# cc-ai/MUNIT

Measured on AMD Instinct MI355X. Metric: images/sec (gen_update+dis_update) @256x256 bs=8, higher is better.
Workload: dtype f32; 1 GPU; config_256.yaml AdaINGen_double+MsImageDis dis_update+gen_update, 256x256, per-GPU batch 8, fp32; global_batch=8, parallelism=dp1, gen_state=1

## Files before the change

### include/munit_hip.h

```cpp
#ifndef MUNIT_HIP_H
#define MUNIT_HIP_H

#include <stddef.h>
#include <stdint.h>

#ifdef __cplusplus
extern "C" {
#endif

typedef void* munit_stream_t;

enum { MUNIT_OK = 0, MUNIT_ERR_ARG = -1, MUNIT_ERR_WORKSPACE = -2, MUNIT_ERR_LAUNCH = -3 };
enum { MUNIT_ACT_NONE = 0, MUNIT_ACT_RELU = 1, MUNIT_ACT_LRELU = 2, MUNIT_ACT_TANH = 3 };
enum { MUNIT_PAD_ZERO = 0, MUNIT_PAD_REFLECT = 1 };
enum { MUNIT_COMPUTE_F32 = 0, MUNIT_COMPUTE_BF16 = 1, MUNIT_COMPUTE_F32X3 = 2 };
enum { MUNIT_DTYPE_F32 = 0, MUNIT_DTYPE_BF16 = 1 };

int munit_version(void);
const char* munit_last_error(void);

typedef void* munit_comm_t;
int munit_comm_unique_id(void* id_out, size_t bytes);
int munit_comm_init(munit_comm_t* comm, int rank, int world, const void* unique_id);
int munit_comm_allreduce(munit_comm_t comm, float* buf, size_t count, munit_stream_t stream);
int munit_comm_destroy(munit_comm_t comm);
int munit_shutdown(void);

int munit_stream_wait_stream(munit_stream_t waiter, munit_stream_t signaler);

typedef struct {
  int B, H, W, Cin;
  int Cout, KH, KW;
  int stride, pad, pad_mode;
  int upsample;
  int act;
  float slope;
  int compute;
  int in_dtype, out_dtype;
} munit_conv_desc;

int munit_conv2d_out_hw(const munit_conv_desc* d, int* Ho, int* Wo);

size_t munit_conv2d_fwd_workspace_bytes(const munit_conv_desc* d);
int munit_conv2d_fwd(const munit_conv_desc* d, const void* x, const float* w, const float* bias,
                     void* y, void* ws, size_t ws_bytes, munit_stream_t stream);

size_t munit_conv2d_dgrad_workspace_bytes(const munit_conv_desc* d);
int munit_conv2d_dgrad(const munit_conv_desc* d, const void* dy, const float* w, const void* add,
                       void* dx, void* ws, size_t ws_bytes, munit_stream_t stream);

size_t munit_conv2d_wgrad_workspace_bytes(const munit_conv_desc* d);
int munit_conv2d_wgrad(const munit_conv_desc* d, const void* x, const void* dy, float* dw,
                       float* db, float beta, void* ws, size_t ws_bytes, munit_stream_t stream);

enum { MUNIT_PASS_FWD = 0, MUNIT_PASS_DGRAD = 1, MUNIT_PASS_WGRAD = 2 };
enum { MUNIT_PREP_NONE = 0, MUNIT_PREP_DGRAD = 1, MUNIT_PREP_SUBPIXEL = 2, MUNIT_PREP_CAST = 3,
       MUNIT_PREP_WINOGRAD = 4, MUNIT_PREP_WINOGRAD_DGRAD = 5, MUNIT_PREP_SUBPIXEL_WINOGRAD = 6,
       MUNIT_PREP_WINOGRAD_S2 = 7, MUNIT_PREP_WINOGRAD_S2_DGRAD = 8,
       MUNIT_PREP_SUBPIXEL_WINOGRAD_DGRAD = 9  };
typedef struct {
  const float* w;
  float* wp;
  int Cout, KH, KW, Cin;
  int kind;
  int ps;
  int bf16;
} munit_prep_item;
size_t munit_conv2d_prepared_weight_bytes(const munit_conv_desc* d, int pass);
int munit_conv2d_prep_item(const munit_conv_desc* d, int pass, const float* w, float* wp, munit_prep_item* out);
int munit_conv2d_prepare_weights(const munit_prep_item* item, munit_stream_t stream);
int munit_conv2d_prepare_weights_batch(const munit_prep_item* items_dev, int n, munit_stream_t stream);
int munit_conv2d_fwd_prepared(const munit_conv_desc* d, const void* x, const float* w, const void* wp,
                              const float* bias, void* y, void* ws, size_t ws_bytes, munit_stream_t stream);
int munit_conv2d_dgrad_prepared(const munit_conv_desc* d, const void* dy, const float* w, const void* wp,
                                const void* add, void* dx, void* ws, size_t ws_bytes, munit_stream_t stream);

size_t munit_linear_workspace_bytes(int B, int K, int N);
int munit_linear_fwd(const float* x, const float* w, const float* bias, float* y, int B, int K, int N, int act,
                     float slope, void* ws, size_t ws_bytes, munit_stream_t stream);
int munit_linear_bwd(const float* x, const float* w, const float* dy, float* dx, float* dw, float* db, int B, int K,
                     int N, float beta, void* ws, size_t ws_bytes, munit_stream_t stream);

double munit_conv2d_executed_flops(const munit_conv_desc* d, int pass);
const char* munit_conv2d_kernel_name(const munit_conv_desc* d, int pass);

int munit_act_bwd(int act, float slope, const float* y, const float* dy, float* dx, size_t n,
                  munit_stream_t stream);

size_t munit_instnorm_workspace_bytes(int B, int HW, int C);
int munit_instnorm_fwd(const float* x, float* y, float* stats, int B, int HW, int C,
                       const float* adain, int ad_ld, int w_off, int b_off, const float* residual,
                       int relu, float eps, void* ws, size_t ws_bytes, munit_stream_t stream);
int munit_instnorm_bwd(const float* x, const float* dy, const float* stats, float* dx, int B, int HW,
                       int C, const float* adain, float* d_adain, int ad_ld, int w_off, int b_off,
                       int relu, void* ws, size_t ws_bytes, munit_stream_t stream);

int munit_instnorm_fwd_bf16(const void* x, void* y, float* stats, int B, int HW, int C,
                            const float* adain, int ad_ld, int w_off, int b_off, const void* residual,
                            int relu, float eps, void* ws, size_t ws_bytes, munit_stream_t stream);
int munit_instnorm_bwd_bf16(const void* x, const void* dy, const float* stats, void* dx, int B, int HW,
                            int C, const float* adain, float* d_adain, int ad_ld, int w_off, int b_off,
                            int relu, void* ws, size_t ws_bytes, munit_stream_t stream);

size_t munit_layernorm_workspace_bytes(int B, int HW, int C);
int munit_layernorm_fwd(const float* x, float* y, float* stats, int B, int HW, int C,
                        const float* gamma, const float* beta, int relu, float eps, void* ws,
                        size_t ws_bytes, munit_stream_t stream);
int munit_layernorm_bwd(const float* x, const float* dy, const float* stats, float* dx, int B, int HW,
                        int C, const float* gamma, const float* beta, float* dgamma, float* dbeta,
                        float acc, int relu, float eps, void* ws, size_t ws_bytes,
                        munit_stream_t stream);

int munit_layernorm_fwd_bf16(const void* x, void* y, float* stats, int B, int HW, int C,
                             const float* gamma, const float* beta, int relu, float eps, void* ws,
                             size_t ws_bytes, munit_stream_t stream);
int munit_layernorm_bwd_bf16(const void* x, const void* dy, const float* stats, void* dx, int B, int HW,
                             int C, const float* gamma, const float* beta, float* dgamma, float* dbeta,
                             float acc, int relu, float eps, void* ws, size_t ws_bytes,
                             munit_stream_t stream);

int munit_avgpool3s2_fwd(const float* x, float* y, int B, int H, int W, int C, munit_stream_t stream);
int munit_avgpool3s2_bwd(const float* dy, float* dx, int B, int H, int W, int C, munit_stream_t stream);
int munit_gap_fwd(const float* x, float* y, int B, int HW, int C, munit_stream_t stream);
int munit_gap_bwd(const float* dy, float* dx, int B, int HW, int C, munit_stream_t stream);

size_t munit_loss_workspace_bytes(size_t n);
int munit_l1_mean_fwd(const float* a, const float* b, const float* mask, size_t npix, int C, float* out,
                      void* ws, size_t ws_bytes, munit_stream_t stream);
int munit_l1_mean_bwd(const float* a, const float* b, const float* mask, size_t npix, int C,
                      const float* gout, float* da, float* db, munit_stream_t stream);
int munit_l1_mean_fwd_bf16(const void* a, const void* b, const float* mask, size_t npix, int C, float* out,
                           void* ws, size_t ws_bytes, munit_stream_t stream);
int munit_l1_mean_bwd_bf16(const void* a, const void* b, const float* mask, size_t npix, int C,
                           const float* gout, void* da, void* db, munit_stream_t stream);
int munit_pair_l1_fwd(const float* x_a, const float* x_b, const float* x_ab, const float* x_ba, size_t npix, int C,
                      float* out, void* ws, size_t ws_bytes, munit_stream_t stream);
int munit_pair_l1_bwd(const float* x_a, const float* x_b, const float* x_ab, const float* x_ba, size_t npix, int C,
                      const float* gout, float* dx_ab, float* dx_ba, munit_stream_t stream);
int munit_mse_const_fwd(const float* x, float target, size_t n, float* out, void* ws, size_t ws_bytes,
                        munit_stream_t stream);
int munit_mse_const_bwd(const float* x, float target, size_t n, const float* gout, float* dx,
                        munit_stream_t stream);
size_t munit_lsgan_workspace_bytes(int nseg);
int munit_lsgan_fwd(const float* const* x, const size_t* n, const float* target, int nseg, float* out, float* seg_out,
                    void* ws, size_t ws_bytes, munit_stream_t stream);
int munit_lsgan_bwd(const float* const* x, const size_t* n, const float* target, int nseg, const float* gout,
                    float* const* dx, munit_stream_t stream);
size_t munit_nsgan_workspace_bytes(int nseg);
int munit_nsgan_fwd(const float* const* x, const size_t* n, const float* target, int nseg, float* out, float* seg_out,
                    void* ws, size_t ws_bytes, munit_stream_t stream);
int munit_nsgan_bwd(const float* const* x, const size_t* n, const float* target, int nseg, const float* gout,
                    float* const* dx, munit_stream_t stream);
int munit_weighted_sum(const float* const* terms, const float* w, int n, float* out,
                       munit_stream_t stream);

int munit_adam_step(float* p, const float* g, float* m, float* v, size_t n, double lr, double beta1,
                    double beta2, double eps, double weight_decay, int step, munit_stream_t stream);

int munit_extraadam_step(float* p, const float* g, float* m, float* v, float* p_saved, size_t n, double lr,
                         double beta1, double beta2, double eps, double weight_decay, int step, int mode,
                         munit_stream_t stream);

int munit_scale(const float* x, float* y, size_t n, float alpha, int accumulate, munit_stream_t stream);

typedef struct {
  long long src_off;
  int src_h, src_w;
  int rs_h, rs_w;
  int crop_i, crop_j;
  int flip;
  int kind;
} munit_image_desc;

int munit_image_ksize(int src_size, int rs_size);
size_t munit_image_preprocess_workspace_bytes(int B, int out_h, int out_w, int ksize_max);
int munit_image_preprocess(const unsigned char* pool, const munit_image_desc* descs, int B, int out_h,
                           int out_w, int ksize_max, float* out, void* ws, size_t ws_bytes,
                           munit_stream_t stream);
// ... 109 lines not shown
```

### munit_amd/_lib.py

```python
import ctypes
import os
from ctypes import POINTER, Structure, c_char_p, c_double, c_float, c_int, c_size_t, c_void_p

_HERE = os.path.dirname(os.path.abspath(__file__))
LIB_PATH = os.environ.get("MUNIT_HIP_LIB") or os.path.join(_HERE, "libmunit_hip.so")

ACT = {"none": 0, "relu": 1, "lrelu": 2, "tanh": 3}
PAD = {"zero": 0, "reflect": 1}
COMPUTE = {"f32": 0, "bf16": 1, "f32x3": 2}
DTYPE = {"f32": 0, "bf16": 1}


class ConvDesc(Structure):
    _fields_ = [("B", c_int), ("H", c_int), ("W", c_int), ("Cin", c_int),
                ("Cout", c_int), ("KH", c_int), ("KW", c_int),
                ("stride", c_int), ("pad", c_int), ("pad_mode", c_int),
                ("upsample", c_int), ("act", c_int), ("slope", c_float), ("compute", c_int),
                ("in_dtype", c_int), ("out_dtype", c_int)]


class PrepItem(Structure):
    _fields_ = [("w", c_void_p), ("wp", c_void_p), ("Cout", c_int), ("KH", c_int), ("KW", c_int), ("Cin", c_int),
                ("kind", c_int), ("ps", c_int), ("bf16", c_int)]


class ImageDesc(Structure):
    _fields_ = [("src_off", ctypes.c_longlong), ("src_h", c_int), ("src_w", c_int), ("rs_h", c_int), ("rs_w", c_int),
                ("crop_i", c_int), ("crop_j", c_int), ("flip", c_int), ("kind", c_int)]


class GemmProblem(Structure):
    _fields_ = [("A", c_void_p), ("B", c_void_p), ("C", c_void_p)]


class GridSrc(Structure):
    _fields_ = [("data", c_void_p), ("n", c_int), ("channels", c_int), ("layout", c_int)]


class RectDesc(Structure):
    _fields_ = [("B", c_int), ("H", c_int), ("W", c_int), ("Cin", c_int), ("x_ld", c_int), ("Cout", c_int), ("y_ld", c_int),
                ("KH", c_int), ("KW", c_int), ("stride", c_int), ("pad_h", c_int), ("pad_w", c_int), ("relu", c_int)]


WINDOW = {"max": 0, "avg": 1}
RECT_TILES = ("128x128", "64x64", "128x64")

_P = c_void_p
_DESC = POINTER(ConvDesc)

SIGNATURES = {
    "munit_version": (c_int, []),
    "munit_last_error": (c_char_p, []),
    "munit_stream_wait_stream": (c_int, [_P, _P]),
    "munit_comm_unique_id": (c_int, [_P, c_size_t]),
    "munit_comm_init": (c_int, [_P, c_int, c_int, _P]),
    "munit_comm_allreduce": (c_int, [_P, _P, c_size_t, _P]),
    "munit_comm_destroy": (c_int, [_P]),
    "munit_shutdown": (c_int, []),
    "munit_conv2d_out_hw": (c_int, [_DESC, POINTER(c_int), POINTER(c_int)]),
    "munit_conv2d_fwd_workspace_bytes": (c_size_t, [_DESC]),
    "munit_conv2d_fwd": (c_int, [_DESC, _P, _P, _P, _P, _P, c_size_t, _P]),
    "munit_conv2d_dgrad_workspace_bytes": (c_size_t, [_DESC]),
    "munit_conv2d_dgrad": (c_int, [_DESC, _P, _P, _P, _P, _P, c_size_t, _P]),
    "munit_conv2d_wgrad_workspace_bytes": (c_size_t, [_DESC]),
    "munit_conv2d_wgrad": (c_int, [_DESC, _P, _P, _P, _P, c_float, _P, c_size_t, _P]),
    "munit_conv2d_prepared_weight_bytes": (c_size_t, [_DESC, c_int]),
    "munit_conv2d_prep_item": (c_int, [_DESC, c_int, _P, _P, POINTER(PrepItem)]),
    "munit_conv2d_prepare_weights": (c_int, [POINTER(PrepItem), _P]),
    "munit_conv2d_prepare_weights_batch": (c_int, [_P, c_int, _P]),
    "munit_conv2d_fwd_prepared": (c_int, [_DESC, _P, _P, _P, _P, _P, _P, c_size_t, _P]),
    "munit_conv2d_dgrad_prepared": (c_int, [_DESC, _P, _P, _P, _P, _P, _P, c_size_t, _P]),
    "munit_conv2d_executed_flops": (c_double, [_DESC, c_int]),
    "munit_conv2d_kernel_name": (c_char_p, [_DESC, c_int]),
    "munit_linear_workspace_bytes": (c_size_t, [c_int, c_int, c_int]),
    "munit_linear_fwd": (c_int, [_P, _P, _P, _P, c_int, c_int, c_int, c_int, c_float, _P, c_size_t, _P]),
    "munit_linear_bwd": (c_int, [_P, _P, _P, _P, _P, _P, c_int, c_int, c_int, c_float, _P, c_size_t, _P]),
    "munit_act_bwd": (c_int, [c_int, c_float, _P, _P, _P, c_size_t, _P]),
    "munit_instnorm_workspace_bytes": (c_size_t, [c_int, c_int, c_int]),
    "munit_instnorm_fwd": (c_int, [_P, _P, _P, c_int, c_int, c_int, _P, c_int, c_int, c_int, _P, c_int,
                                   c_float, _P, c_size_t, _P]),
    "munit_instnorm_bwd": (c_int, [_P, _P, _P, _P, c_int, c_int, c_int, _P, _P, c_int, c_int, c_int, c_int,
                                   _P, c_size_t, _P]),
    "munit_instnorm_fwd_bf16": (c_int, [_P, _P, _P, c_int, c_int, c_int, _P, c_int, c_int, c_int, _P, c_int,
                                        c_float, _P, c_size_t, _P]),
    "munit_instnorm_bwd_bf16": (c_int, [_P, _P, _P, _P, c_int, c_int, c_int, _P, _P, c_int, c_int, c_int, c_int,
                                        _P, c_size_t, _P]),
    "munit_layernorm_workspace_bytes": (c_size_t, [c_int, c_int, c_int]),
    "munit_layernorm_fwd": (c_int, [_P, _P, _P, c_int, c_int, c_int, _P, _P, c_int, c_float, _P, c_size_t, _P]),
    "munit_layernorm_bwd": (c_int, [_P, _P, _P, _P, c_int, c_int, c_int, _P, _P, _P, _P, c_float, c_int,
                                    c_float, _P, c_size_t, _P]),
    "munit_layernorm_fwd_bf16": (c_int, [_P, _P, _P, c_int, c_int, c_int, _P, _P, c_int, c_float, _P, c_size_t, _P]),
    "munit_layernorm_bwd_bf16": (c_int, [_P, _P, _P, _P, c_int, c_int, c_int, _P, _P, _P, _P, c_float, c_int,
                                         c_float, _P, c_size_t, _P]),
    "munit_avgpool3s2_fwd": (c_int, [_P, _P, c_int, c_int, c_int, c_int, _P]),
    "munit_avgpool3s2_bwd": (c_int, [_P, _P, c_int, c_int, c_int, c_int, _P]),
    "munit_gap_fwd": (c_int, [_P, _P, c_int, c_int, c_int, _P]),
    "munit_gap_bwd": (c_int, [_P, _P, c_int, c_int, c_int, _P]),
    "munit_loss_workspace_bytes": (c_size_t, [c_size_t]),
    "munit_l1_mean_fwd": (c_int, [_P, _P, _P, c_size_t, c_int, _P, _P, c_size_t, _P]),
    "munit_l1_mean_bwd": (c_int, [_P, _P, _P, c_size_t, c_int, _P, _P, _P, _P]),
    "munit_l1_mean_fwd_bf16": (c_int, [_P, _P, _P, c_size_t, c_int, _P, _P, c_size_t, _P]),
    "munit_l1_mean_bwd_bf16": (c_int, [_P, _P, _P, c_size_t, c_int, _P, _P, _P, _P]),
    "munit_pair_l1_fwd": (c_int, [_P, _P, _P, _P, c_size_t, c_int, _P, _P, c_size_t, _P]),
    "munit_pair_l1_bwd": (c_int, [_P, _P, _P, _P, c_size_t, c_int, _P, _P, _P, _P]),
    "munit_mse_const_fwd": (c_int, [_P, c_float, c_size_t, _P, _P, c_size_t, _P]),
    "munit_mse_const_bwd": (c_int, [_P, c_float, c_size_t, _P, _P, _P]),
    "munit_lsgan_workspace_bytes": (c_size_t, [c_int]),
    "munit_lsgan_fwd": (c_int, [POINTER(c_void_p), POINTER(c_size_t), POINTER(c_float), c_int, _P, _P, _P, c_size_t, _P]),
    "munit_lsgan_bwd": (c_int, [POINTER(c_void_p), POINTER(c_size_t), POINTER(c_float), c_int, _P, POINTER(c_void_p), _P]),
    "munit_nsgan_workspace_bytes": (c_size_t, [c_int]),
    "munit_nsgan_fwd": (c_int, [POINTER(c_void_p), POINTER(c_size_t), POINTER(c_float), c_int, _P, _P, _P, c_size_t, _P]),
    "munit_nsgan_bwd": (c_int, [POINTER(c_void_p), POINTER(c_size_t), POINTER(c_float), c_int, _P, POINTER(c_void_p), _P]),
    "munit_weighted_sum": (c_int, [POINTER(c_void_p), POINTER(c_float), c_int, _P, _P]),
    "munit_adam_step": (c_int, [_P, _P, _P, _P, c_size_t, c_double, c_double, c_double, c_double, c_double, c_int,
                                _P]),
    "munit_extraadam_step": (c_int, [_P, _P, _P, _P, _P, c_size_t, c_double, c_double, c_double, c_double,
                                     c_double, c_int, c_int, _P]),
    "munit_scale": (c_int, [_P, _P, c_size_t, c_float, c_int, _P]),
    "munit_image_ksize": (c_int, [c_int, c_int]),
    "munit_image_preprocess_workspace_bytes": (c_size_t, [c_int, c_int, c_int, c_int]),
    "munit_image_preprocess": (c_int, [_P, _P, c_int, c_int, c_int, c_int, _P, _P, c_size_t, _P]),
    "munit_mask_preprocess_workspace_bytes": (c_size_t, [c_int, c_int, c_int]),
    "munit_mask_preprocess": (c_int, [_P, _P, c_int, c_int, c_int, _P, _P, c_size_t, _P]),
    "munit_label_preprocess_workspace_bytes": (c_size_t, [c_int, c_int, c_int]),
    "munit_label_preprocess": (c_int, [_P, _P, c_int, c_int, c_int, _P, _P, c_size_t, _P]),
    "munit_image_grid_workspace_bytes": (c_size_t, [c_int, c_int, c_int, c_int]),
    "munit_image_grid_u8": (c_int, [POINTER(GridSrc), c_int, c_int, c_int, c_int, c_float, c_float, _P, _P, c_size_t, _P]),
    "munit_seg_input_fwd": (c_int, [_P, _P, c_size_t, _P]),
    "munit_seg_input_bwd": (c_int, [_P, _P, c_size_t, _P]),
    "munit_space_to_batch": (c_int, [_P, _P, c_int, c_int, c_int, c_int, c_int, c_int, _P]),
    "munit_maxpool3s2_fwd": (c_int, [_P, _P, _P, c_int, c_int, c_int, c_int, _P]),
    "munit_maxpool3s2_bwd": (c_int, [_P, _P, _P, c_int, c_int, c_int, c_int, _P]),
    "munit_add_relu_fwd": (c_int, [_P, _P, _P, c_size_t, _P]),
    "munit_seg_ce_workspace_bytes": (c_size_t, [c_int, c_int, c_int, c_int]),
    "munit_seg_ce_fwd": (c_int, [_P, _P, _P, c_int, c_int, c_int, c_int, c_float, _P, _P, c_size_t, _P]),
    "munit_seg_ce_bwd": (c_int, [_P, _P, _P, c_int, c_int, c_int, c_int, c_float, _P, _P, _P, c_size_t, _P]),
    "munit_seg_ce_gt_fwd": (c_int, [_P, _P, _P, c_int, c_int, c_int, c_int, c_float, _P, _P, c_size_t, _P]),
    "munit_seg_ce_gt_bwd": (c_int, [_P, _P, _P, c_int, c_int, c_int, c_int, c_float, _P, _P, _P, c_size_t, _P]),
    "munit_seg_labels": (c_int, [_P, c_int, c_int, c_int, c_int, _P, _P]),
    "munit_seg_ce_direct_workspace_bytes": (c_size_t, [c_int, c_int, c_int, c_int, c_int]),
    "munit_seg_ce_direct_fwd": (c_int, [_P, _P, c_int, c_int, c_int, c_int, c_int, c_float, _P, _P, c_size_t, _P]),
    "munit_seg_ce_direct_bwd": (c_int, [_P, _P, c_int, c_int, c_int, c_int, c_int, c_float, _P, _P, _P, c_size_t, _P]),
    "munit_avgpool7_fwd": (c_int, [_P, _P, c_int, c_int, c_int, c_int, _P]),
    "munit_avgpool7_bwd": (c_int, [_P, _P, c_int, c_int, c_int, c_int, _P]),
    "munit_batchnorm_workspace_bytes": (c_size_t, [c_int]),
    "munit_batchnorm_fwd": (c_int, [_P, _P, _P, _P, _P, _P, ctypes.c_longlong, c_int, _P, _P, c_int, c_int, c_float, c_float,
                                    _P, c_size_t, _P]),
    "munit_batchnorm_bwd": (c_int, [_P, _P, _P, _P, _P, _P, _P, _P, _P, c_float, ctypes.c_longlong, c_int, c_int, _P,
                                    c_size_t, _P]),
    "munit_batchnorm_dp_workspace_bytes": (c_size_t, [c_int]),
    "munit_batchnorm_dp_stats_local": (c_int, [_P, ctypes.c_longlong, c_int, c_int, c_int, _P, c_size_t, _P, c_size_t, _P]),
    "munit_batchnorm_dp_fwd_apply": (c_int, [_P, _P, _P, _P, _P, _P, ctypes.c_longlong, c_int, c_int, _P, c_size_t, _P, _P,
                                             c_int, c_float, c_float, _P]),
    "munit_batchnorm_dp_bwd_local": (c_int, [_P, _P, _P, _P, _P, ctypes.c_longlong, c_int, c_int, c_int, c_int, _P, c_size_t,
                                             _P, c_size_t, _P]),
    "munit_batchnorm_dp_bwd_finish": (c_int, [_P, _P, _P, _P, _P, _P, _P, _P, _P, c_float, ctypes.c_longlong, c_int, c_int,
                                              c_int, c_int, _P, c_size_t, _P, c_size_t, _P]),
    "munit_maxpool2_fwd": (c_int, [_P, _P, _P, c_int, c_int, c_int, c_int, _P]),
    "munit_maxpool2_bwd": (c_int, [_P, _P, _P, c_int, c_int, c_int, c_int, _P]),
    "munit_avgpool16_fwd": (c_int, [_P, _P, c_int, c_int, c_int, c_int, _P]),
    "munit_avgpool16_bwd": (c_int, [_P, _P, c_int, c_int, c_int, c_int, _P]),
# ... 43 lines not shown
```

### munit_amd/csrc/norm.hip

```cpp
#include "common.h"

namespace {

constexpr int NT = 256;
constexpr int MAX_SPLIT = 64;
constexpr int MAX_NORM_C = 4 * NT;

constexpr float NORM_LRELU_SLOPE = 0.2f;
__device__ inline float norm_act(float v, int act) {
  if (act == MUNIT_ACT_RELU) return v > 0.f ? v : 0.f;
  if (act == MUNIT_ACT_LRELU) return v > 0.f ? v : v * NORM_LRELU_SLOPE;
  if (act == MUNIT_ACT_TANH) return tanhf(v);
  return v;
}
__device__ inline float norm_act_grad(float pre, float g, int act) {
  if (act == MUNIT_ACT_RELU) return pre > 0.f ? g : 0.f;
  if (act == MUNIT_ACT_LRELU) return pre > 0.f ? g : g * NORM_LRELU_SLOPE;
  if (act == MUNIT_ACT_TANH) { const float t = tanhf(pre); return g * (1.f - t * t); }
  return g;
}

struct Lay {
  int CQ;
  int QB;
// ... 310 lines not shown
    const float rstd = (float)(1.0 / sqrt(var + (double)eps));
    float w = 1.f, bb = 0.f;
    if (adain != nullptr) {
      w = adain[(long long)b * ad_ld + w_off + c];
      bb = adain[(long long)b * ad_ld + b_off + c];
    }
    if (sp == 0) {
      stats[((long long)b * C + c) * 2] = mean;
      stats[((long long)b * C + c) * 2 + 1] = rstd;
    }
    scale[threadIdx.x] = rstd * w;
    shift[threadIdx.x] = bb - mean * rstd * w;
  }
  __syncthreads();
  const int per = (HW + nsplit - 1) / nsplit;
  const int p0 = sp * per, p1 = min(HW, p0 + per);
  const long long base = (long long)b * HW * C + c0;
  const int q = threadIdx.x & 15;
  const f32x4 sc = *reinterpret_cast<const f32x4*>(scale + q * 4);
  const f32x4 sh = *reinterpret_cast<const f32x4*>(shift + q * 4);
#pragma unroll 4
  for (int p = p0 + (threadIdx.x >> 4); p < p1; p += NT / 16) {
    const long long o = base + (long long)p * C + q * 4;
    f32x4 v = ld4(x + o);
    v = v * sc + sh;
    if (relu) {
#pragma unroll
      for (int e = 0; e < 4; ++e) v[e] = norm_act(v[e], relu);
    }
    if (residual != nullptr) v += ld4(residual + o);
    st4(y + o, v);
  }
}

template <typename T>
__global__ __launch_bounds__(NT) void in_bwd_apply_sliced_kernel(const T* __restrict__ x, const T* __restrict__ dy,
                                                                 const double* __restrict__ partial,
                                                                 const float* __restrict__ stats, T* __restrict__ dx, int HW,
                                                                 int C, int nsplit, const float* __restrict__ adain,
                                                                 float* __restrict__ d_adain, int ad_ld, int w_off, int b_off,
                                                                 int relu) {
  __shared__ double red[3][SLICE][2];
  __shared__ __attribute__((aligned(16))) float s_co[6][SLICE];
  const int b = blockIdx.y, sp = blockIdx.x, c0 = blockIdx.z * SLICE;
  double a1, a2;
  fold_slice(partial, b, C, nsplit, c0, red, a1, a2);
  if (threadIdx.x < SLICE) {
    const int c = c0 + threadIdx.x;
    if (d_adain != nullptr && sp == 0) {
      d_adain[(long long)b * ad_ld + w_off + c] = (float)a2;
      d_adain[(long long)b * ad_ld + b_off + c] = (float)a1;
    }
    const double inv_n = 1.0 / (double)HW;
    s_co[0][threadIdx.x] = stats[((long long)b * C + c) * 2];
    s_co[1][threadIdx.x] = stats[((long long)b * C + c) * 2 + 1];
    s_co[2][threadIdx.x] = adain ? adain[(long long)b * ad_ld + w_off + c] : 1.f;
    s_co[3][threadIdx.x] = adain ? adain[(long long)b * ad_ld + b_off + c] : 0.f;
    s_co[4][threadIdx.x] = (float)(a1 * inv_n);
    s_co[5][threadIdx.x] = (float)(a2 * inv_n);
  }
  __syncthreads();
  const int per = (HW + nsplit - 1) / nsplit;
  const int p0 = sp * per, p1 = min(HW, p0 + per);
  const long long base = (long long)b * HW * C + c0;
  const int q = threadIdx.x & 15;
  const f32x4 mean = *reinterpret_cast<const f32x4*>(&s_co[0][q * 4]);
  const f32x4 rstd = *reinterpret_cast<const f32x4*>(&s_co[1][q * 4]);
  const f32x4 w = *reinterpret_cast<const f32x4*>(&s_co[2][q * 4]);
  const f32x4 bb = *reinterpret_cast<const f32x4*>(&s_co[3][q * 4]);
  const f32x4 a1v = *reinterpret_cast<const f32x4*>(&s_co[4][q * 4]);
  const f32x4 a2v = *reinterpret_cast<const f32x4*>(&s_co[5][q * 4]);
#pragma unroll 4
  for (int p = p0 + (threadIdx.x >> 4); p < p1; p += NT / 16) {
    const long long o = base + (long long)p * C + q * 4;
    const f32x4 xv = ld4(x + o);
    const f32x4 xh = (xv - mean) * rstd;
    f32x4 g = ld4(dy + o);
    if (relu) {
#pragma unroll
      for (int e = 0; e < 4; ++e) g[e] = norm_act_grad(xv[e] * (rstd[e] * w[e]) + (bb[e] - mean[e] * rstd[e] * w[e]), g[e], relu);
    }
    const f32x4 r = rstd * w * (g - a1v - xh * a2v);
    st4(dx + o, r);
  }
}

__device__ inline double block_sum(double v, double* red) {
#pragma unroll
  for (int off = 32; off > 0; off >>= 1) v += __shfl_xor(v, off, 64);
  const int w = threadIdx.x >> 6;
  __syncthreads();
  if ((threadIdx.x & 63) == 0) red[w] = v;
  __syncthreads();
  double t = 0.0;
#pragma unroll
  for (int i = 0; i < NT / 64; ++i) t += red[i];
  return t;
}

template <typename T>
__global__ __launch_bounds__(NT) void ln_stats_kernel(const T* __restrict__ x, double* __restrict__ partial,
                                                      long long n_per_sample, int nsplit) {
  __shared__ double red[NT / 64];
  const int b = blockIdx.y, sp = blockIdx.x;
  const T* xb = x + (long long)b * n_per_sample;
  const long long nq = n_per_sample >> 2;
  const long long per = (nq + nsplit - 1) / nsplit;
  const long long q0 = sp * per, q1 = min(nq, q0 + per);
  const float piv = ld1(xb);
  double s1 = 0.0, s2 = 0.0;
  for (long long i = q0 + threadIdx.x; i < q1; i += NT) {
    f32x4 v = ld4(xb + i * 4);
#pragma unroll
    for (int e = 0; e < 4; ++e) {
      double d = (double)(v[e] - piv);
      s1 += d;
      s2 += d * d;
    }
  }
  s1 = block_sum(s1, red);
  s2 = block_sum(s2, red);
  if (threadIdx.x == 0) {
    partial[((long long)b * nsplit + sp) * 2] = s1;
    partial[((long long)b * nsplit + sp) * 2 + 1] = s2;
  }
}

template <typename T>
__device__ inline void ln_finish(const double* partial, const T* xb, int b, int nsplit, long long n,
                                 float* mean, float* sigma) {
  double s1 = 0.0, s2 = 0.0;
  for (int k = 0; k < nsplit; ++k) {
    s1 += partial[((long long)b * nsplit + k) * 2];
    s2 += partial[((long long)b * nsplit + k) * 2 + 1];
  }
  const double d = s1 / (double)n;
  double var = (s2 - s1 * d) / (double)(n - 1);
  if (var < 0.0) var = 0.0;
  *mean = (float)((double)ld1(xb) + d);
  *sigma = (float)sqrt(var);
}

template <typename T>
__global__ __launch_bounds__(NT) void ln_apply_kernel(const T* __restrict__ x, T* __restrict__ y,
                                                      const double* __restrict__ partial, float* __restrict__ stats,
                                                      int HW, int C, int nsplit, const float* __restrict__ gamma,
                                                      const float* __restrict__ beta, int relu, float eps) {
  extern __shared__ float sm[];
  float* scale = sm;
  float* shift = sm + C;
  const int b = blockIdx.y, sp = blockIdx.x;
  const long long n = (long long)HW * C;
  const T* xb = x + (long long)b * n;
  float mean, sigma;
  ln_finish(partial, xb, b, nsplit, n, &mean, &sigma);
  const float inv = 1.f / (sigma + eps);
  if (sp == 0 && threadIdx.x == 0) {
    stats[b * 2] = mean;
    stats[b * 2 + 1] = sigma;
  }
  for (int c = threadIdx.x; c < C; c += NT) {
    scale[c] = inv * gamma[c];
    shift[c] = beta[c] - mean * inv * gamma[c];
  }
  __syncthreads();
  const int CQ = C >> 2;
// ... 62 lines not shown
    __syncthreads();
    if (pl == 0) {
      for (int l = 1; l < L.PL; ++l) {
        const double* d = sm + ((l * L.QB + q) * 8);
#pragma unroll
        for (int e = 0; e < 4; ++e) { s1[e] += d[e]; s2[e] += d[4 + e]; }
      }
      double* o = cpart + ((long long)(b * nsplit + sp) * 2) * C + qq * 4;
#pragma unroll
      for (int e = 0; e < 4; ++e) { o[e] = s1[e]; o[C + e] = s2[e]; }
    }
    __syncthreads();
  }
  t1 = block_sum(t1, red);
  t2 = block_sum(t2, red);
  if (threadIdx.x == 0) {
    spart[((long long)b * nsplit + sp) * 2] = t1;
    spart[((long long)b * nsplit + sp) * 2 + 1] = t2;
  }
}

template <typename T>
__global__ __launch_bounds__(NT) void ln_bwd_apply_kernel(const T* __restrict__ x, const T* __restrict__ dy,
                                                          const float* __restrict__ stats,
                                                          const double* __restrict__ spart, T* __restrict__ dx,
                                                          int HW, int C, int nsplit, const float* __restrict__ gamma,
                                                          const float* __restrict__ beta, int relu, float eps) {
  const int b = blockIdx.y, sp = blockIdx.x;
  const long long n = (long long)HW * C;
  const float mean = stats[b * 2];
  const float sigma = stats[b * 2 + 1];
  const float inv = 1.f / (sigma + eps);
  double S1 = 0.0, S2 = 0.0;
  for (int k = 0; k < nsplit; ++k) {
    S1 += spart[((long long)b * nsplit + k) * 2];
    S2 += spart[((long long)b * nsplit + k) * 2 + 1];
  }
  const float c1 = (float)(S1 / (double)n);
  const float c2 = sigma > 0.f ? (float)(S2 / ((double)(n - 1) * (double)sigma)) : 0.f;
  const int CQ = C >> 2;
  const long long nq = n >> 2;
  const long long per = (nq + nsplit - 1) / nsplit;
  const long long q0 = sp * per, q1 = min(nq, q0 + per);
  const long long base = (long long)b * n;
  for (long long i = q0 + threadIdx.x; i < q1; i += NT) {
    const int q = (int)(i % CQ);
    const f32x4 gm = *reinterpret_cast<const f32x4*>(gamma + q * 4);
    const f32x4 bt = *reinterpret_cast<const f32x4*>(beta + q * 4);
    const f32x4 xv = ld4(x + base + i * 4);
    const f32x4 xn = (xv - mean) * inv;
    f32x4 g = ld4(dy + base + i * 4);
    if (relu) {
#pragma unroll
      for (int e = 0; e < 4; ++e) g[e] = norm_act_grad(xv[e] * (inv * gm[e]) + (bt[e] - mean * inv * gm[e]), g[e], relu);
    }
    const f32x4 r = (g * gm - c1) * inv - xn * c2;
    st4(dx + base + i * 4, r);
  }
}

__global__ __launch_bounds__(NT) void ln_bwd_param_kernel(const double* __restrict__ cpart, float* __restrict__ dgamma,
                                                          float* __restrict__ dbeta, int C, int nblk, float acc) {
  __shared__ double red[NT / 64];
  const int c = blockIdx.x;
  double g = 0.0, bt = 0.0;
  for (int k = threadIdx.x; k < nblk; k += NT) {
    g += cpart[((long long)k * 2) * C + c];
    bt += cpart[((long long)k * 2 + 1) * C + c];
  }
  g = block_sum(g, red);
  bt = block_sum(bt, red);
  if (threadIdx.x == 0) {
    dgamma[c] = (acc != 0.f ? acc * dgamma[c] : 0.f) + (float)g;
    dbeta[c] = (acc != 0.f ? acc * dbeta[c] : 0.f) + (float)bt;
  }
}

}

namespace {
size_t in_partial_bytes(int B, int C) { return align_up((size_t)B * MAX_SPLIT * 2 * C * sizeof(double), 256); }
bool in_sliced(int C) { return C % SLICE == 0 && !MUNIT_ENV_FLAG("MUNIT_DEBUG_NO_SLICED_NORM"); }
int sliced_split(int B, int HW, int C) { return std::max(1, pick_split(B, HW) / (C / SLICE)); }
}
extern "C" size_t munit_instnorm_workspace_bytes(int B, int HW, int C) {
  return in_partial_bytes(B, C) + align_up((size_t)B * 6 * C * sizeof(float), 256);
}

namespace {
template <typename T>
int instnorm_fwd_t(const T* x, T* y, float* stats, int B, int HW, int C, const float* adain, int ad_ld, int w_off,
                   int b_off, const T* residual, int relu, float eps, void* ws, size_t ws_bytes, munit_stream_t stream) {
  MUNIT_CHECK_ARG(x && y && stats && ws, "instnorm_fwd: null pointer");
  MUNIT_CHECK_ARG(B > 0 && HW > 0 && C > 0 && C % 4 == 0, "instnorm_fwd: bad dims B=%d HW=%d C=%d", B, HW, C);
  MUNIT_CHECK_ARG(C <= MAX_NORM_C, "instnorm_fwd: C=%d too large", C);
  if (ws_bytes < munit_instnorm_workspace_bytes(B, HW, C)) {
    munit_set_error("instnorm_fwd: workspace too small");
    return MUNIT_ERR_WORKSPACE;
  }
  hipStream_t st = (hipStream_t)stream;
  double* partial = reinterpret_cast<double*>(ws);
  if (in_sliced(C)) {
    const int ns = sliced_split(B, HW, C);
    const Lay Ls = make_lay(SLICE);
    hipLaunchKernelGGL(in_stats_kernel<T>, dim3(ns, B, C / SLICE), dim3(NT), (size_t)Ls.PL * Ls.QB * 8 * sizeof(double), st, x,
                       partial, HW, C, ns, SLICE);
    MUNIT_CHECK_LAUNCH("in_stats");
    hipLaunchKernelGGL(in_apply_sliced_kernel<T>, dim3(ns, B, C / SLICE), dim3(NT), 0, st, x, y, partial, stats, HW, C, ns, adain,
                       ad_ld, w_off, b_off, eps, residual, relu);
    MUNIT_CHECK_LAUNCH("in_apply_sliced");
    return MUNIT_OK;
  }
  const int ns = pick_split(B, HW);
  const Lay L = make_lay(C);
  hipLaunchKernelGGL(in_stats_kernel<T>, dim3(ns, B), dim3(NT), (size_t)L.PL * L.QB * 8 * sizeof(double), st, x,
                     partial, HW, C, ns, C);
  MUNIT_CHECK_LAUNCH("in_stats");
  float* coef = reinterpret_cast<float*>(reinterpret_cast<char*>(ws) + in_partial_bytes(B, C));
  hipLaunchKernelGGL(in_finalize_kernel<T>, dim3(cdiv(C, 64), B), dim3(NT), 0, st, x, partial, stats, coef, B,
                     HW, C, ns, adain, ad_ld, w_off, b_off, eps);
  MUNIT_CHECK_LAUNCH("in_finalize");
  hipLaunchKernelGGL(in_apply_kernel<T>, dim3(ns, B), dim3(NT), (size_t)2 * C * sizeof(float), st, x, y, coef, HW, C,
                     ns, residual, relu);
  MUNIT_CHECK_LAUNCH("in_apply");
  return MUNIT_OK;
}

template <typename T>
int instnorm_bwd_t(const T* x, const T* dy, const float* stats, T* dx, int B, int HW, int C, const float* adain,
                   float* d_adain, int ad_ld, int w_off, int b_off, int relu, void* ws, size_t ws_bytes,
                   munit_stream_t stream) {
  MUNIT_CHECK_ARG(x && dy && stats && dx && ws, "instnorm_bwd: null pointer");
  MUNIT_CHECK_ARG(B > 0 && HW > 0 && C > 0 && C % 4 == 0 && C <= MAX_NORM_C, "instnorm_bwd: bad dims");
  if (ws_bytes < munit_instnorm_workspace_bytes(B, HW, C)) {
    munit_set_error("instnorm_bwd: workspace too small");
    return MUNIT_ERR_WORKSPACE;
  }
  hipStream_t st = (hipStream_t)stream;
  double* partial = reinterpret_cast<double*>(ws);
  if (in_sliced(C)) {
    const int ns = sliced_split(B, HW, C);
    const Lay Ls = make_lay(SLICE);
    hipLaunchKernelGGL(in_bwd_stats_kernel<T>, dim3(ns, B, C / SLICE), dim3(NT), (size_t)Ls.PL * Ls.QB * 8 * sizeof(double), st, x,
                       dy, stats, partial, HW, C, ns, adain, ad_ld, w_off, b_off, relu, SLICE);
    MUNIT_CHECK_LAUNCH("in_bwd_stats");
    hipLaunchKernelGGL(in_bwd_apply_sliced_kernel<T>, dim3(ns, B, C / SLICE), dim3(NT), 0, st, x, dy, partial, stats, dx, HW, C, ns,
                       adain, d_adain, ad_ld, w_off, b_off, relu);
    MUNIT_CHECK_LAUNCH("in_bwd_apply_sliced");
    return MUNIT_OK;
  }
  const int ns = pick_split(B, HW);
  const Lay L = make_lay(C);
  hipLaunchKernelGGL(in_bwd_stats_kernel<T>, dim3(ns, B), dim3(NT), (size_t)L.PL * L.QB * 8 * sizeof(double), st, x,
                     dy, stats, partial, HW, C, ns, adain, ad_ld, w_off, b_off, relu, C);
  MUNIT_CHECK_LAUNCH("in_bwd_stats");
  float* coef = reinterpret_cast<float*>(reinterpret_cast<char*>(ws) + in_partial_bytes(B, C));
  hipLaunchKernelGGL(in_bwd_finalize_kernel, dim3(cdiv(C, 64), B), dim3(NT), 0, st, partial, stats, coef, B, HW,
                     C, ns, adain, d_adain, ad_ld, w_off, b_off);
  MUNIT_CHECK_LAUNCH("in_bwd_finalize");
  hipLaunchKernelGGL(in_bwd_apply_kernel<T>, dim3(ns, B), dim3(NT), (size_t)6 * C * sizeof(float), st, x, dy, coef, dx,
                     HW, C, ns, relu);
  MUNIT_CHECK_LAUNCH("in_bwd_apply");
  return MUNIT_OK;
}
}

extern "C" int munit_instnorm_fwd(const float* x, float* y, float* stats, int B, int HW, int C,
                                  const float* adain, int ad_ld, int w_off, int b_off, const float* residual,
                                  int relu, float eps, void* ws, size_t ws_bytes, munit_stream_t stream) {
  return instnorm_fwd_t<float>(x, y, stats, B, HW, C, adain, ad_ld, w_off, b_off, residual, relu, eps, ws, ws_bytes, stream);
}
extern "C" int munit_instnorm_fwd_bf16(const void* x, void* y, float* stats, int B, int HW, int C,
                                       const float* adain, int ad_ld, int w_off, int b_off, const void* residual,
                                       int relu, float eps, void* ws, size_t ws_bytes, munit_stream_t stream) {
  return instnorm_fwd_t<bf16_t>(reinterpret_cast<const bf16_t*>(x), reinterpret_cast<bf16_t*>(y), stats, B, HW, C, adain, ad_ld,
                                w_off, b_off, reinterpret_cast<const bf16_t*>(residual), relu, eps, ws, ws_bytes, stream);
}
extern "C" int munit_instnorm_bwd(const float* x, const float* dy, const float* stats, float* dx, int B, int HW,
                                  int C, const float* adain, float* d_adain, int ad_ld, int w_off, int b_off,
                                  int relu, void* ws, size_t ws_bytes, munit_stream_t stream) {
  return instnorm_bwd_t<float>(x, dy, stats, dx, B, HW, C, adain, d_adain, ad_ld, w_off, b_off, relu, ws, ws_bytes, stream);
}
extern "C" int munit_instnorm_bwd_bf16(const void* x, const void* dy, const float* stats, void* dx, int B, int HW,
                                       int C, const float* adain, float* d_adain, int ad_ld, int w_off, int b_off,
// ... 88 lines not shown
```

Baseline: 79.14 images/s.

## Add single-kernel register-resident instance norm forward for small f32 planes

Adds a one-pass instance-norm forward kernel for f32. Each block handles 16 channels of one image, holds the spatial values in registers, computes shifted double-precision sums, reduces them in shared memory and applies the scale/shift, ReLU and residual in the same launch. This replaces the separate stats and apply kernels, removing one launch and a second read of x when the plane fits. It also adds a route query function. The cost is heavy register use (16 f32x4 per thread) and use only where the split and HW limits hold.

```diff
diff --git a/include/munit_hip.h b/include/munit_hip.h
--- a/include/munit_hip.h
+++ b/include/munit_hip.h
@@ -94,6 +94,8 @@
 int munit_instnorm_bwd(const float* x, const float* dy, const float* stats, float* dx, int B, int HW,
                        int C, const float* adain, float* d_adain, int ad_ld, int w_off, int b_off,
                        int relu, void* ws, size_t ws_bytes, munit_stream_t stream);
+
+int munit_instnorm_route(int B, int HW, int C, int dtype);
 
 int munit_instnorm_fwd_bf16(const void* x, void* y, float* stats, int B, int HW, int C,
                             const float* adain, int ad_ld, int w_off, int b_off, const void* residual,
diff --git a/munit_amd/_lib.py b/munit_amd/_lib.py
--- a/munit_amd/_lib.py
+++ b/munit_amd/_lib.py
@@ -77,6 +77,7 @@
     "munit_linear_bwd": (c_int, [_P, _P, _P, _P, _P, _P, c_int, c_int, c_int, c_float, _P, c_size_t, _P]),
     "munit_act_bwd": (c_int, [c_int, c_float, _P, _P, _P, c_size_t, _P]),
     "munit_instnorm_workspace_bytes": (c_size_t, [c_int, c_int, c_int]),
+    "munit_instnorm_route": (c_int, [c_int, c_int, c_int, c_int]),
     "munit_instnorm_fwd": (c_int, [_P, _P, _P, c_int, c_int, c_int, _P, c_int, c_int, c_int, _P, c_int,
                                    c_float, _P, c_size_t, _P]),
     "munit_instnorm_bwd": (c_int, [_P, _P, _P, _P, c_int, c_int, c_int, _P, _P, c_int, c_int, c_int, c_int,
diff --git a/munit_amd/csrc/norm.hip b/munit_amd/csrc/norm.hip
--- a/munit_amd/csrc/norm.hip
+++ b/munit_amd/csrc/norm.hip
@@ -416,6 +416,146 @@
     }
     const f32x4 r = rstd * w * (g - a1v - xh * a2v);
     st4(dx + o, r);
+  }
+}
+
+constexpr int OP_CH = 16;
+constexpr int OP_Q = OP_CH / 4;
+constexpr int OP_PL = 16;
+constexpr int OP_NV = 16;
+constexpr int OP_MAX_SPLIT = 16;
+constexpr int OP_TPS = OP_PL * OP_Q;
+constexpr int OP_NT = OP_TPS * OP_MAX_SPLIT;
+constexpr int OP_LINE = 32 / OP_CH;
+static_assert(OP_TPS == 4 * OP_CH, "onepass_fold: four split groups of OP_CH threads in the smallest block");
+
+__device__ inline void onepass_block(int C, int& b, int& c0) {
+  constexpr int GRP = 8 * OP_LINE;
+  const int i = blockIdx.x, grp = i / GRP, r = i % GRP;
+  const bool full = (grp + 1) * GRP <= (int)gridDim.x;
+  const int cg = grp * GRP + (full ? ((r & 7) * OP_LINE + (r >> 3)) : r);
+  const int G = C / OP_CH;
+  b = cg / G;
+  c0 = (cg % G) * OP_CH;
+}
+
+__device__ inline void onepass_lanes(const double (&v1)[4], const double (&v2)[4], double* __restrict__ lane,
+                                     double (*part)[2][OP_CH], double* __restrict__ partial, int b, int C, int nsplit, int c0) {
+  const int s = threadIdx.x / OP_TPS, ln = threadIdx.x % OP_TPS;
+  double* mine = lane + (s * OP_PL) * OP_CH;
+#pragma unroll
+  for (int which = 0; which < 2; ++which) {
+#pragma unroll
+    for (int e = 0; e < 4; ++e) mine[ln * 4 + e] = which ? v2[e] : v1[e];
+    __syncthreads();
+    if (ln < OP_CH) {
+      double a = mine[ln];
+      for (int l = 1; l < OP_PL; ++l) a += mine[l * OP_CH + ln];
+      partial[((long long)(b * nsplit + s) * 2 + which) * C + c0 + ln] = a;
+      part[s][which][ln] = a;
+    }
+    __syncthreads();
+  }
+}
+
+__device__ inline void onepass_fold(const double (*part)[2][OP_CH], int nsplit, double (*red)[OP_CH][2], double& s1, double& s2) {
+  const int cl = threadIdx.x % OP_CH, g = threadIdx.x / OP_CH;
+  s1 = 0.0;
+  s2 = 0.0;
+  if (g < 4) {
+    for (int k = g; k < nsplit; k += 4) {
+      s1 += part[k][0][cl];
+      s2 += part[k][1][cl];
+    }
+    if (g > 0) {
+      red[g - 1][cl][0] = s1;
+      red[g - 1][cl][1] = s2;
+    }
+  }
+  __syncthreads();
+  if (g == 0) {
+#pragma unroll
+    for (int j = 0; j < 3; ++j) {
+      s1 += red[j][cl][0];
+      s2 += red[j][cl][1];
+    }
+  }
+}
+
+__global__ __launch_bounds__(OP_NT) void in_onepass_kernel(const float* __restrict__ x, float* __restrict__ y,
+                                                           double* __restrict__ partial, float* __restrict__ stats, int HW,
+                                                           int C, int nsplit, const float* __restrict__ adain, int ad_ld,
+                                                           int w_off, int b_off, float eps,
+                                                           const float* __restrict__ residual, int relu) {
+  __shared__ double lane[OP_MAX_SPLIT * OP_PL * OP_CH];
+  __shared__ double part[OP_MAX_SPLIT][2][OP_CH];
+  __shared__ double red[3][OP_CH][2];
+  __shared__ __attribute__((aligned(16))) float scale[OP_CH], shift[OP_CH];
+  int b, c0;
+  onepass_block(C, b, c0);
+  const int s = threadIdx.x / OP_TPS, pl = (threadIdx.x % OP_TPS) / OP_Q, q = threadIdx.x % OP_Q;
+  const int per = (HW + nsplit - 1) / nsplit;
+  const int p0 = s * per + pl, p1 = min(HW, s * per + per);
+  const long long plane = (long long)b * HW * C + c0;
+  const unsigned to = (unsigned)(p0 * C + q * 4);
+  const float* xb = x + plane;
+  const float* rb = residual != nullptr ? residual + plane : nullptr;
+  f32x4 v[OP_NV];
+#pragma unroll
+  for (int j = 0; j < OP_NV; ++j) {
+    const int p = p0 + OP_PL * j;
+    v[j] = p < p1 ? ld4(xb + j * OP_PL * C + to) : f32x4{0.f, 0.f, 0.f, 0.f};
+  }
+  const f32x4 piv = ld4(xb + q * 4);
+  double s1[4] = {0, 0, 0, 0}, s2[4] = {0, 0, 0, 0};
+#pragma unroll
+  for (int j = 0; j < OP_NV; ++j) {
+    if (p0 + OP_PL * j < p1) {
+      const f32x4 d = v[j] - piv;
+#pragma unroll
+      for (int e = 0; e < 4; ++e) {
+        s1[e] += (double)d[e];
+        s2[e] += (double)d[e] * (double)d[e];
+      }
+    }
+  }
+  onepass_lanes(s1, s2, lane, part, partial, b, C, nsplit, c0);
+  double t1, t2;
+  onepass_fold(part, nsplit, red, t1, t2);
+  if (threadIdx.x < OP_CH) {
+    const int c = c0 + threadIdx.x;
+    const double inv_n = 1.0 / (double)HW;
+    const double d = t1 * inv_n;
+    const float mean = (float)((double)x[plane + threadIdx.x] + d);
+    double var = t2 * inv_n - d * d;
+    var = var > 0.0 ? var : 0.0;
+    const float rstd = (float)(1.0 / sqrt(var + (double)eps));
+    float w = 1.f, bb = 0.f;
+    if (adain != nullptr) {
+      w = adain[(long long)b * ad_ld + w_off + c];
+      bb = adain[(long long)b * ad_ld + b_off + c];
+    }
+    stats[((long long)b * C + c) * 2] = mean;
+    stats[((long long)b * C + c) * 2 + 1] = rstd;
+    scale[threadIdx.x] = rstd * w;
+    shift[threadIdx.x] = bb - mean * rstd * w;
+  }
+  __syncthreads();
+  const f32x4 sc = *reinterpret_cast<const f32x4*>(scale + q * 4);
+  const f32x4 sh = *reinterpret_cast<const f32x4*>(shift + q * 4);
+  float* yb = y + plane;
+#pragma unroll
+  for (int j = 0; j < OP_NV; ++j) {
+    const int p = p0 + OP_PL * j;
+    if (p < p1) {
+      f32x4 r = v[j] * sc + sh;
+      if (relu) {
+#pragma unroll
+        for (int e = 0; e < 4; ++e) r[e] = norm_act(r[e], relu);
+      }
+      if (rb != nullptr) r += ld4(rb + j * OP_PL * C + to);
+      st4(yb + j * OP_PL * C + to, r);
+    }
   }
 }
 
@@ -644,6 +784,16 @@
 size_t in_partial_bytes(int B, int C) { return align_up((size_t)B * MAX_SPLIT * 2 * C * sizeof(double), 256); }
 bool in_sliced(int C) { return C % SLICE == 0 && !MUNIT_ENV_FLAG("MUNIT_DEBUG_NO_SLICED_NORM"); }
 int sliced_split(int B, int HW, int C) { return std::max(1, pick_split(B, HW) / (C / SLICE)); }
+int onepass_split(int B, int HW, int C, bool f32) {
+  if (!f32 || !in_sliced(C) || MUNIT_ENV_FLAG("MUNIT_DEBUG_NO_ONEPASS_NORM")) return 0;
+  const int ns = sliced_split(B, HW, C);
+  return (ns <= OP_MAX_SPLIT && cdiv(HW, ns) <= OP_PL * OP_NV) ? ns : 0;
+}
+}
+extern "C" int munit_instnorm_route(int B, int HW, int C, int dtype) {
+  if (B <= 0 || HW <= 0 || C <= 0 || C % 4 != 0 || C > MAX_NORM_C) return -1;
+  if (onepass_split(B, HW, C, dtype == MUNIT_DTYPE_F32)) return 2;
+  return in_sliced(C) ? 1 : 0;
 }
 extern "C" size_t munit_instnorm_workspace_bytes(int B, int HW, int C) {
   return in_partial_bytes(B, C) + align_up((size_t)B * 6 * C * sizeof(float), 256);
@@ -662,6 +812,14 @@
   }
   hipStream_t st = (hipStream_t)stream;
   double* partial = reinterpret_cast<double*>(ws);
+  if constexpr (std::is_same<T, float>::value) {
+    if (const int ns = onepass_split(B, HW, C, true)) {
+      hipLaunchKernelGGL(in_onepass_kernel, dim3(B * (C / OP_CH)), dim3(OP_TPS * ns), 0, st, x, y, partial, stats, HW, C, ns, adain,
+                         ad_ld, w_off, b_off, eps, residual, relu);
+      MUNIT_CHECK_LAUNCH("in_onepass");
+      return MUNIT_OK;
+    }
+  }
   if (in_sliced(C)) {
     const int ns = sliced_split(B, HW, C);
     const Lay Ls = make_lay(SLICE);
```

Result: faster. 80.08 images/s (median of 6 runs) (+1.2%).
